# ESMS-Group-Public/FoKL-GPy

Hardware: AMD Instinct MI355X
Metric: candidate-terms/sec (basis build + Gibbs + BIC) (higher is better)
Workload: dtype f64

## Files before the change

fokl_gpy_amd/_capi.py:

```python
import ctypes
import os

import numpy as np

_HERE = os.path.dirname(os.path.abspath(__file__))
LIB_PATH = os.environ.get('FOKL_HIP_LIBRARY', os.path.join(_HERE, 'libfokl_hip.so'))

UNIQUE_ID_BYTES = 128
K_BASIS, K_GRAM, K_RESID, K_PREDICT, K_RESID_MF, K_GRAM_MFMA, K_GRAM_REDUCE = 0, 1, 2, 3, 4, 5, 6
K_INTEGRATE, K_BAND = 7, 8
K_OPTIMIZE = 9
K_OPTIMIZE_SYSTEM = 10
K_POPULATION = 11
K_RESAMPLE = 12
K_SCORE = 13
K_INFER = 14
K_DESIGN = 15
INTEGRATE_MAX_STATES = 4
RESID_TERMS_MAX_FACTORS = 32
RESID_TERMS_MAX_ORDER = 8
RESID_TERMS_LAYOUTS = ((8, 1), (16, 1), (8, 2), (4, 4), (2, 8), (8, 4), (16, 2), (4, 8))
SLOT_ONES, SLOT_Y, SLOT_FIRST_FREE = 0, 1, 2
PREDICT_NONE, PREDICT_VALU_LDS, PREDICT_VALU_GLOBAL, PREDICT_MFMA = 0, 1, 2, 3
POPULATION_COEFFICIENTS = ('none', 'registers', 'table')
# ... 106 lines not shown
    'fokl_stream_given_gauss': (c_dbl, [c_vp]),
    'fokl_stream_destroy': (None, [c_vp]),
    'fokl_stream_walk': (c_int, [c_vp, c_int, c_int, c_dbl, c_dbl, c_vp, c_vp, c_vp, c_vp]),
    'fokl_stream_tell': (c_int, [c_vp, c_vp]),
    'fokl_stream_seek': (c_int, [c_vp, c_vp]),
    'fokl_stream_hold': (c_int, [c_vp, c_vp]),
    'fokl_stream_release': (c_int, [c_vp, ctypes.c_uint64]),
    'fokl_stream_advance_floor': (c_int, [c_vp]),
    'fokl_stream_state': (c_int, [c_vp, c_vp, c_vp, c_vp, c_vp]),
    'fokl_stream_expand': (c_int, [c_vp, c_int, c_dbl, c_dbl, c_vp, c_int, c_int, c_vp, c_vp, c_vp, c_vp, c_vp]),
    'fokl_stream_stats': (c_int, [c_vp, c_vp, c_vp, c_vp, c_vp, c_vp]),
    'fokl_stream_set_helpers': (c_int, [c_vp, c_int, c_vp]),
    'fokl_stream_place_bulk': (c_int, [c_vp, c_vp, c_int]),
    'fokl_stream_fast_ln_error': (c_dbl, [c_i64]),
    'fokl_search_create': (c_int, [c_vp, c_vp, c_vp, c_vp]),
    'fokl_search_bind_spectral': (c_int, [c_vp, c_vp, c_int, c_dbl, c_int]),
    'fokl_search_hold_spectral': (c_int, [c_vp, c_int]),
    'fokl_search_set_update': (c_int, [c_vp, c_int, c_int, c_int]),
    'fokl_search_set_decide': (c_int, [c_vp, c_int, c_dbl]),
    'fokl_search_set_deterministic': (c_int, [c_vp, c_int]),
    'fokl_search_destroy': (None, [c_vp]),
    'fokl_search_error': (ctypes.c_char_p, [c_vp]),
    'fokl_search_mispredicted': (c_int, [c_vp]),
    'fokl_search_set_substage': (c_int, [c_vp, c_vp, c_int]),
    'fokl_search_speculate': (c_int, [c_vp, c_vp, c_vp, c_int]),
    'fokl_search_drop_speculation': (c_int, [c_vp]),
    'fokl_search_spectral': (c_int, [c_vp, c_vp, c_int, c_vp, c_int, c_vp]),
    'fokl_search_spectral_from': (c_int, [c_vp, c_vp, c_int, c_vp, c_int, c_vp, c_int, c_vp]),
    'fokl_spectrum_done': (c_int, [c_vp]),
    'fokl_spectrum_wait': (c_int, [c_vp, c_vp, c_vp, c_vp]),
    'fokl_spectrum_release': (None, [c_vp, c_vp]),
    'fokl_spectrum_retain': (c_int, [c_vp, c_vp]),
    'fokl_search_model_begin': (c_int, [c_vp, c_vp, c_int, c_vp, c_int, c_vp, c_vp, c_vp, c_int, c_vp, c_vp]),
    'fokl_search_model_commit': (c_int, [c_vp, c_vp, c_vp, c_dbl, c_int, c_vp]),
    'fokl_run_create': (c_int, [c_vp, c_vp, c_vp]),
    'fokl_run_set_update': (c_int, [c_vp, c_int, c_int, c_int]),
    'fokl_run_search': (c_int, [c_vp, c_vp]),
    'fokl_run_result': (c_int, [c_vp, c_vp, c_vp, c_vp, c_vp, c_vp]),
    'fokl_run_arrays': (c_int, [c_vp, c_vp, c_vp, c_vp, c_vp, c_vp, c_vp]),
    'fokl_run_error': (ctypes.c_char_p, [c_vp]),
    'fokl_run_destroy': (None, [c_vp]),
    'fokl_search_score': (c_int, [c_vp, c_vp, c_dbl, c_dbl, c_int, c_int, c_vp]),
    'fokl_outcome_info': (c_int, [c_vp, c_vp, c_vp]),
    'fokl_outcome_spectrum': (c_int, [c_vp, c_vp, c_vp]),
    'fokl_outcome_chain_ready': (c_int, [c_vp]),
    'fokl_outcome_draws': (c_int, [c_vp, c_vp, c_vp]),
    'fokl_outcome_intercept_scale': (c_int, [c_vp, c_vp, c_vp]),
    'fokl_outcome_new_term_stats': (c_int, [c_vp, c_vp, c_vp, c_int, c_int, c_int, c_vp, c_vp]),
    'fokl_outcome_release': (None, [c_vp, c_vp]),
    'fokl_outcome_drop': (None, [c_vp, c_vp]),
    'fokl_search_verify': (c_int, [c_vp, c_int]),
    'fokl_search_register_forecast': (c_int, [c_vp, c_vp, c_int, c_vp, c_dbl]),
    'fokl_search_clear_forecasts': (None, [c_vp]),
    'fokl_search_likely_first_tests': (c_int, [c_vp, c_vp, c_int, c_dbl, c_vp, c_vp, c_vp]),
    'fokl_search_stats': (c_int, [c_vp, c_vp, c_int]),
    'fokl_search_trace': (c_i64, [c_vp, c_vp, c_i64]),
    'fokl_search_kill_tests': (c_int, [c_vp, c_vp, c_vp]),
    'fokl_finish_tape_blocks': (c_int, [c_int, c_int, c_vp, c_vp, c_vp, c_vp, c_int, c_int, c_int, c_vp]),
    'fokl_gibbs_chain_from_finished_tape': (c_int, [c_vp, c_vp, c_int, c_dbl, c_dbl, c_dbl, c_dbl, c_dbl, c_int, c_vp,
                                                    c_vp, c_vp, c_vp, c_int, c_vp, c_vp, c_vp, c_vp]),
    'fokl_gibbs_chain_segments_host': (c_int, [c_vp, c_vp, c_int, c_dbl, c_dbl, c_dbl, c_dbl, c_dbl, c_int, c_vp, c_vp,
                                               c_vp, c_vp, c_int, c_vp, c_vp, c_vp, c_vp, c_int, c_int, c_vp]),
    'fokl_rng_normals': (c_int, [c_vp, c_vp, c_vp, c_vp, c_i64, c_vp]),
    'fokl_rng_gammas': (c_int, [c_vp, c_vp, c_vp, c_vp, c_dbl, c_dbl, c_i64, c_vp]),
    'fokl_gp_integrate': (c_int, [c_int, c_int, c_i64, c_vp, c_vp, c_vp, c_vp, c_vp, c_vp, c_vp, c_vp, c_vp, c_int, c_int,
                                  c_dbl, c_vp, c_vp]),
    'fokl_gp_integrate_ensemble': (c_int, [c_vp, c_int, c_int, c_int, c_i64, c_vp, c_vp, c_vp, c_vp, c_vp, c_vp, c_vp, c_vp,
                                           c_vp, c_vp, c_int, c_int, c_dbl, c_vp, c_int, c_int, c_vp, c_vp, c_vp]),
    'fokl_simulate_ensemble': (c_int, [c_vp, c_vp, c_int, c_vp, c_vp, c_vp, c_vp]),
    'fokl_simulate_report': (c_int, [c_vp, c_vp]),
    'fokl_simulate_adaptive': (c_int, [c_vp, c_vp, c_int, c_dbl, c_vp, c_int, c_int, c_vp, c_vp, c_vp, c_vp, c_vp, c_vp, c_vp, c_vp, c_vp,
                                       c_vp]),
# ... 1276 lines not shown
        mean_w, flag = job.wait()
        return job.fetch_w(), np.array(mean_w), bool(flag[0])
    finally:
        job.release()



_OPS_SIGS = (('reserve_slots', [c_vp, c_int]),
             ('build_terms', [c_vp, c_vp, c_int, c_vp]),
             ('gram', [c_vp, c_vp, c_int, c_vp, c_int, c_vp, c_int, c_int]),
             ('gram_launch', [c_vp, c_vp, c_int, c_vp, c_int, c_int]),
             ('gram_fetch', [c_vp, c_vp, c_i64]),
             ('gram_ready', [c_vp]),
             ('bic_resid', [c_vp, c_vp, c_int, c_vp, c_vp, c_int]),
             ('bic_resid_launch', [c_vp, c_vp, c_int, c_vp]),
             ('bic_resid_fetch', [c_vp, c_vp, c_int]),
             ('bic_resid_terms_launch', [c_vp, c_vp, c_int, c_vp]))
_OPS_TYPES = {name: ctypes.CFUNCTYPE(c_int, *args) for name, args in _OPS_SIGS}


class _BackendOps(ctypes.Structure):
    _fields_ = [('ctx', c_vp)] + [(name, c_vp) for name, _ in _OPS_SIGS] + [('kernel_id', c_i32)]


class _RunParams(ctypes.Structure):
    _fields_ = [(name, c_i32) for name in (
        'm', 'n_phis', 'way3', 'tolerance', 'gimmie', 'draws', 'half0', 'lookahead', 'lookahead_native', 'foresight',
        'speculate_across', 'forecast_early', 'forecast_polls', 'matrix_free', 'update_from', 'update_depth',
        'update_lookahead', 'head_start', 'slot_capacity')]


RUN_STATS = ('terms_physical', 'substages', 'forecasts_used', 'forecasts_early', 'resid_matrix_free', 't_resid',
             'phase_prepare', 'phase_model', 'phase_statistics', 'phase_tests', 'phase_wrap_up')


def backend_ops(backend, kernel_id):
    lib = load()
    ops = _BackendOps()
    ops.kernel_id = int(kernel_id)
    ctx = getattr(backend, 'ctx', None)
    if isinstance(ctx, DeviceContext):
        ops.ctx = ctx._h
        for name, _ in _OPS_SIGS:
            setattr(ops, name, ctypes.cast(getattr(lib, 'fokl_' + name), c_vp).value)
        return ops, (ctx,)
    pending, raised = {}, []

    def arr(ptr, count, ctype, dtype):
        return np.array(np.ctypeslib.as_array(ctypes.cast(ptr, ctypes.POINTER(ctype * count)).contents), dtype=dtype)

    def guard(fn):
        def call(*args):
            try:
                fn(*args)
                return 0
            except BaseException as exc:
                raised.append(exc)
                return -3
        return call

    def out(ptr, values):
        values = np.ascontiguousarray(values, dtype=np.float64).reshape(-1)
        ctypes.memmove(ptr, values.ctypes.data, values.nbytes)

    def reserve_slots(_c, n):
        backend.reserve_slots(int(n))

    def build_terms(_c, terms, T, slots):
        sl = arr(slots, T, ctypes.c_int32, np.int32)
        m = pending['m']
        backend.build_terms(arr(terms, T * m, ctypes.c_int32, np.int32).reshape(T, m), [int(v) for v in sl])

    def gram(_c, rows, nr, cols, nc, dst, _path, allreduce):
        out(dst, backend.gram([int(v) for v in arr(rows, nr, ctypes.c_int32, np.int32)],
                              [int(v) for v in arr(cols, nc, ctypes.c_int32, np.int32)], bool(allreduce)))

    def gram_launch(_c, rows, nr, cols, nc, allreduce):
        pending['gram'] = backend.gram([int(v) for v in arr(rows, nr, ctypes.c_int32, np.int32)],
                                       [int(v) for v in arr(cols, nc, ctypes.c_int32, np.int32)], bool(allreduce))

    def gram_fetch(_c, dst, count):
        block = pending.pop('gram')
        assert block.size == count
        out(dst, block)

    def bic_resid(_c, slots, nc, betahat, dst, allreduce):
        out(dst, backend.bic_resid([int(v) for v in arr(slots, nc, ctypes.c_int32, np.int32)],
                                   arr(betahat, nc, ctypes.c_double, np.float64), bool(allreduce)))

    def bic_resid_launch(_c, slots, nc, betahat):
        pending['resid'] = backend.bic_resid([int(v) for v in arr(slots, nc, ctypes.c_int32, np.int32)],
                                             arr(betahat, nc, ctypes.c_double, np.float64), False)

    def bic_resid_fetch(_c, dst, _allreduce):
        out(dst, pending.pop('resid'))

    table = dict(reserve_slots=reserve_slots, build_terms=build_terms, gram=gram, gram_launch=gram_launch,
                 gram_fetch=gram_fetch, bic_resid=bic_resid, bic_resid_launch=bic_resid_launch,
                 bic_resid_fetch=bic_resid_fetch)
    keep = [pending, raised]
    for name, fn in table.items():
        cb = _OPS_TYPES[name](guard(fn))
        keep.append(cb)
        setattr(ops, name, ctypes.cast(cb, c_vp).value)
    return ops, tuple(keep)


class NativeRun:

    def __init__(self, backend, kernel_id, **params):
        self._lib = load()
        self._h = None
        self._ops, self._keep = backend_ops(backend, kernel_id)
        if isinstance(self._keep[0], dict):
            self._keep[0]['m'] = int(params['m'])
        self._prm = _RunParams(**{k: int(v) for k, v in params.items()})
        self.m = int(params['m'])
        h = c_vp(0)
        _check(self._lib.fokl_run_create(ctypes.byref(self._ops), ctypes.byref(self._prm), ctypes.byref(h)))
        self._h = h
        self._reraise()

    def _reraise(self):
        raised = self._keep[1] if isinstance(self._keep[0], dict) else None
        if raised:
            exc = raised[0]
            del raised[:]
            raise exc

    def set_update(self, from_columns, depth, lookahead):
        _check(self._lib.fokl_run_set_update(self._h, int(from_columns), int(depth), int(lookahead)))

    def search(self, native_search):
        rc = self._lib.fokl_run_search(self._h, native_search._h)
        self._reraise()
        if rc != 0:
            native_search._checked(rc)
        return self

    def result(self):
        rows, n_evs, subs = c_i32(0), c_i32(0), c_i32(0)
        best, last = c_vp(0), c_vp(0)
        _check(self._lib.fokl_run_result(self._h, ctypes.byref(rows), ctypes.byref(n_evs), ctypes.byref(subs),
                                         ctypes.byref(best), ctypes.byref(last)))
        mtx = np.zeros((max(rows.value, 0), self.m), dtype=np.int32)
        evs = np.zeros(n_evs.value)
        sizes = np.zeros(max(subs.value, 1), dtype=np.int32)
        stats = np.zeros(16)
        total = self._lib.fokl_run_arrays(self._h, _ptr(mtx) if mtx.size else None, _ptr(evs) if evs.size else None,
                                          _ptr(sizes), None, None, _ptr(stats))
        mean_abs, rel_std = np.zeros(max(total, 1)), np.zeros(max(total, 1))
        self._lib.fokl_run_arrays(self._h, None, None, None, _ptr(mean_abs), _ptr(rel_std), None)
        per, at = [], 0
        for size in sizes[:subs.value]:
            per.append(dict(mean_abs=mean_abs[at:at + size].copy(), rel_std=rel_std[at:at + size].copy()))
            at += int(size)
        return (mtx.astype(np.float64), evs, per, best.value, last.value, dict(zip(RUN_STATS, stats[:len(RUN_STATS)])))

    def close(self):
        if self._h is not None and self._h:
            self._lib.fokl_run_destroy(self._h)
            self._h = None

    def __del__(self):
        try:
            self.close()
        except Exception:
            pass


class _FirstTrialStruct(ctypes.Structure):
    _fields_ = [(name, ctypes.c_void_p) for name in ('trial', 'slope', 'moved', 'pooled', 'ft', 'ft_sums', 'phi_t', 'a_t', 'z',
                                                      'status', 'descent')]


class _SystemStruct(ctypes.Structure):
    _fields_ = [('n_members', c_int), ('n_states', c_int), ('n_steps', c_i64), ('h', c_dbl), ('n_forcing_cols', c_int),
                ('forcing', c_vp), ('n_norm_forcing', c_int), ('n_norm', c_int), ('norm_src', c_vp), ('norm_lo', c_vp),
                ('norm_span', c_vp), ('n_forcing_factors', c_int), ('n_factors', c_int), ('fac_norm', c_vp), ('fac_kind', c_vp),
                ('fac_row', c_vp), ('fac_degree', c_vp), ('n_spline_rows', c_int), ('spline_table', c_vp), ('n_bern_rows', c_int),
                ('bern_table', c_vp), ('n_entries', c_int), ('entries', c_vp), ('entry_begin', c_vp), ('entry_count', c_vp),
                ('constant', c_vp), ('n_coef', c_int), ('coef', c_vp), ('y0', c_vp), ('box', c_vp)]


class _ControlProblemStruct(ctypes.Structure):
    _fields_ = [('n_controls', c_int), ('n_segments', c_int), ('seg_first', c_vp), ('norm_control', c_vp), ('ctl_lo', c_vp),
                ('ctl_width', c_vp), ('ref', c_vp), ('track_weight', c_vp), ('terminal_weight', c_vp), ('limit_lo', c_vp),
                ('limit_hi', c_vp), ('limit_weight', c_dbl), ('move_weight', c_vp), ('previous', c_vp), ('has_previous', c_int),
                ('n_starts', c_int), ('z0', c_vp), ('max_iter', c_int), ('tol', c_dbl)]

# ... 933 lines not shown
```

fokl_gpy_amd/csrc/fokl_run.cpp:

```cpp
#include <algorithm>
#include <chrono>
#include <cmath>
#include <cstdint>
#include <cstring>
#include <map>
#include <memory>
#include <string>
#include <vector>

#include "../../include/fokl_hip_internal.h"

extern void fokl_set_global_error(const std::string &msg);

namespace {

inline double now_s()
{
    return 1e-9 * (double)std::chrono::duration_cast<std::chrono::nanoseconds>(
                      std::chrono::steady_clock::now().time_since_epoch())
                      .count();
}

using Gram = std::shared_ptr<std::vector<double>>;

// ... 134 lines not shown
    for (int r = 0; r < vm; ++r) {
        const double *b = block.data() + (size_t)r * block_ld;
        double *row = o + (size_t)(n_prev + r) * L;
        for (int j = 0; j < n_prev; ++j) {
            const double v = b[block_kept[(size_t)j]];
            row[j] = v;
            o[(size_t)j * L + n_prev + r] = v;
        }
        for (int c = 0; c < vm; ++c) row[n_prev + c] = b[over + c];
        row[A2] = o[(size_t)A2 * L + n_prev + r] = b[over + vm];
    }
    return out;
}

}

struct fokl_run {
    fokl_backend_ops ops{};
    fokl_run_params prm{};
    Slots pool;
    Patterns patterns;
    std::vector<double> base;
    Ahead ahead;
    bool have_next = false;
    int next_stage = 0;
    std::vector<int32_t> next_indvec;
    std::vector<int32_t> mtx;
    int mtx_rows = 0;
    std::vector<double> evs;
    fokl_outcome *best_model = nullptr, *last_model = nullptr;
    std::vector<double> stat_mean_abs, stat_rel_std;
    std::vector<int32_t> stat_sizes;
    double stats[FOKL_RUN_STATS] = {};
    std::string error;
};

namespace {

int run_fail(fokl_run *r, int code, const std::string &msg)
{
    if (r) r->error = msg;
    fokl_set_global_error(msg);
    return code;
}

enum RunStat {
    R_TERMS_PHYSICAL, R_SUBSTAGES, R_FORECASTS_USED, R_FORECASTS_EARLY, R_RESID_MATRIX_FREE, R_T_RESID, R_PHASE_PREPARE,
    R_PHASE_MODEL, R_PHASE_STATISTICS, R_PHASE_TESTS, R_PHASE_WRAP_UP, R_COUNT
};
static_assert(R_COUNT <= FOKL_RUN_STATS, "fokl_run_stats: grow FOKL_RUN_STATS");

int matrix_free_pay_from(const fokl_backend_ops &ops, const std::vector<int32_t> &terms, int rows, int m)
{
    static const int layouts[8][2] = {{8, 1}, {16, 1}, {8, 2}, {4, 4}, {2, 8}, {8, 4}, {16, 2}, {4, 8}};
    if (!ops.bic_resid_terms_launch || rows < 1) return -1;
    int max_order = 0;
    for (int t = 0; t < rows; ++t) {
        int nz = 0;
        for (int j = 0; j < m; ++j) {
            const int v = terms[(size_t)t * m + j];
            nz += v != 0;
            max_order = std::max(max_order, v);
        }
        if (nz > 2) return -1;
    }
    if (max_order == 0) return -1;
    if (ops.kernel_id != 0 && max_order > 8) return -1;
    int inputs = 0, deepest = 0;
    for (int j = 0; j < m; ++j) {
        std::vector<int32_t> seen;
        for (int t = 0; t < rows; ++t) {
            const int v = terms[(size_t)t * m + j];
            if (v != 0 && std::find(seen.begin(), seen.end(), v) == seen.end()) seen.push_back(v);
        }
        inputs += !seen.empty();
        deepest = std::max(deepest, (int)seen.size());
    }
    int best = -1;
    for (auto &l : layouts)
        if (inputs <= l[0] && deepest <= l[1] && (best < 0 || l[0] * l[1] < best)) best = l[0] * l[1];
    if (best < 0) return -1;
    return ops.kernel_id != 0 ? 0 : (int)(3.5 * best);
}

static const bool g_build_at_start = !(std::getenv("FOKL_BUILD_AHEAD_AT") && std::strcmp(std::getenv("FOKL_BUILD_AHEAD_AT"), "model") == 0);

struct Loop {
    fokl_run *r;
    fokl_search *s;
    const fokl_backend_ops &ops;
    const fokl_run_params &prm;
    int m;
    std::vector<int32_t> damtx;
    std::vector<int32_t> model_slots;
    std::vector<int> keep;
    Gram gram;
    int gram_A = 0;
    std::vector<int32_t> active_slots;
    int A = 0, vm = 0, n_prev = 0, vm_next = -1;
    Gram cur;
    std::vector<int32_t> terms_arr;
    int terms_pay_from = 0;
    std::map<std::vector<int64_t>, int64_t> term_ids;
    std::vector<SpectrumRef> early;
    std::vector<std::vector<int32_t>> early_keys;
    std::vector<int32_t> predicted_kills;
    bool have_predicted = false;
    Ahead ahead;
    bool have_coming = false;
    int coming_stage = 0;
    std::vector<int32_t> coming_indvec;
    struct Forecast {
        std::vector<int32_t> key;
        SpectrumRef sp;
    };
    std::vector<Forecast> forecasts;
    std::vector<fokl_outcome *> outcomes, retiring;
    int rc_cb = FOKL_OK;

    Loop(fokl_run *run, fokl_search *search) : r(run), s(search), ops(run->ops), prm(run->prm), m(run->prm.m) {}

    void release(SpectrumRef &sp)
    {
        if (sp.h) fokl_spectrum_release(s, sp.h);
        sp.h = nullptr;
        sp.gram.reset();
    }

    std::vector<int32_t> columns_without(int count, const std::vector<int32_t> &removed) const
    {
        std::vector<int32_t> out;
        for (int c = 0; c < count; ++c)
            if (std::find(removed.begin(), removed.end(), c) == removed.end()) out.push_back(c);
        return out;
    }

    int fetch_block(Ahead &a)
    {
        if (a.pending) {
            const int nc = a.over + a.T + 1;
            a.block.resize((size_t)a.T * nc);
            const int rc = ops.gram_fetch(ops.ctx, a.block.data(), (int64_t)a.T * nc);
            if (rc != FOKL_OK) return rc;
            a.pending = false;
        }
        return FOKL_OK;
    }

    int build_ahead(const std::vector<int32_t> &indvec, const std::vector<int32_t> &active, Ahead *out)
    {
        Ahead a;
// ... 243 lines not shown
                return rc;
            std::vector<int> kept((size_t)n_prev);
            for (int i = 0; i < n_prev; ++i) kept[(size_t)i] = i;
            cur = extend_gram(*gram, gram_A, keep, block, T, (int)cols.size(), kept, n_prev);
        }
        vm = (int)(vecs.size() / (size_t)m);
        damtx.insert(damtx.end(), vecs.begin(), vecs.end());
        const int dam = (int)(damtx.size() / (size_t)m);
        if ((rc = set_active_terms()) != FOKL_OK) return rc;
        active_slots.assign(1, FOKL_SLOT_ONES);
        active_slots.insert(active_slots.end(), model_slots.begin(), model_slots.end());
        active_slots.insert(active_slots.end(), new_slots.begin(), new_slots.end());
        A = (int)active_slots.size();
        vm_next = have_coming ? (int)(arrangements(coming_indvec).size() / (size_t)m) : -1;
        early.clear();
        early_keys.clear();
        have_predicted = false;
        bool guessed = false;
        std::vector<std::pair<int, bool>> then;
        if (vm > 0 && A > 1) then.push_back({A - 1, false});
        if (prm.lookahead > 0 && spectral_job.h && fokl_spectrum_done(spectral_job.h)) {
            if ((rc = guess_first_tests(spectral_job.h, vm, NAN, true, &then)) != FOKL_OK) return rc;
            guessed = true;
        }
        lap(R_PHASE_PREPARE);

        std::vector<int32_t> idx((size_t)A);
        for (int i = 0; i < A; ++i) idx[(size_t)i] = i;
        std::vector<int32_t> then_sizes, then_model;
        for (auto &p : then) {
            then_sizes.push_back(p.first);
            then_model.push_back(p.second ? 1 : 0);
        }
        fokl_spectrum *spectrum = nullptr;
        fokl_tape *tape = nullptr;
        if ((rc = fokl_search_model_begin(s, cur->data(), A + 1, idx.data(), A, spectral_job.h, then_sizes.data(),
                                          then_model.data(), (int)then_sizes.size(), &spectrum, &tape)) != FOKL_OK)
            return rc;
        if (g_build_at_start && have_coming && prm.foresight > 0) {
            if ((rc = build_ahead_columns(coming_indvec, &ahead)) != FOKL_OK) {
                fokl_spectrum_release(s, spectrum);
                return rc;
            }
        }
        const double *buffer = nullptr;
        int p1_check = 0;
        if ((rc = fokl_spectrum_wait(s, spectrum, &buffer, &p1_check)) != FOKL_OK) {
            fokl_spectrum_release(s, spectrum);
            return rc;
        }
        const double *betahat = buffer + 2 * (size_t)A;
        if (!terms_arr.empty() && A >= terms_pay_from) {
            rc = ops.bic_resid_terms_launch(ops.ctx, terms_arr.data() + m, A - 1, betahat);
            R->stats[R_RESID_MATRIX_FREE] += 1;
        } else {
            rc = ops.bic_resid_launch(ops.ctx, active_slots.data(), A, betahat);
        }
        if (rc == FOKL_OK && ahead.built && !ahead.valid) rc = launch_ahead_gram(active_slots, &ahead);
        if (rc == FOKL_OK && !guessed && prm.lookahead > 0 && vm > 0) {
            rc = guess_first_tests(spectrum, vm, NAN, false);
            guessed = rc == FOKL_OK;
        }
        fokl_outcome *full = nullptr;
        if (rc == FOKL_OK) rc = fokl_search_model_commit(s, spectrum, tape, (*cur)[(size_t)A * (A + 1) + A], vm, &full);
        if (rc != FOKL_OK) {
            fokl_spectrum_release(s, spectrum);
            return rc;
        }
        release(spectral_job);
        outcomes.push_back(full);
        auto forecast_now = [&]() {
            if (!(g_build_at_start && prm.forecast_early && ahead.valid && ahead.pending && have_predicted && ops.gram_ready &&
                  forecasts.empty()))
                return;
            if (!ops.gram_ready(ops.ctx)) return;
            foresee(predicted_kills.data(), (int)predicted_kills.size());
            if (rc_cb == FOKL_OK) R->stats[R_FORECASTS_EARLY] += 1;
        };
        forecast_now();
        if (rc_cb != FOKL_OK) return rc_cb;
        {
            const double t0 = now_s();
            double mom[2] = {0, 0};
            if ((rc = ops.bic_resid_fetch(ops.ctx, mom, 0)) != FOKL_OK) return rc;
            R->stats[R_T_RESID] += now_s() - t0;
            forecast_now();
            if (rc_cb != FOKL_OK) return rc_cb;
            double ev_model = 0;
            if ((rc = fokl_search_score(s, full, mom[0], mom[1], n_prev, 0, &ev_model)) != FOKL_OK) return rc;
        }
        fokl_outcome *best = full;
        fokl_outcome_view view{};
        if ((rc = fokl_outcome_info(s, full, &view)) != FOKL_OK) return rc;
        double ev = view.ev;
        lap(R_PHASE_MODEL);

        if (!guessed && prm.lookahead > 0) {
            fokl_spectrum *own = nullptr;
            if ((rc = fokl_outcome_spectrum(s, full, &own)) != FOKL_OK) return rc;
            rc = guess_first_tests(own, vm, view.siglik, false);
            fokl_spectrum_release(s, own);
            if (rc != FOKL_OK) return rc;
        }
        release_retired();
        if (have_coming && prm.foresight > 0 && !ahead.valid && !ahead.built) {
            if ((rc = build_ahead(coming_indvec, active_slots, &ahead)) != FOKL_OK) return rc;
        }
        if (prm.forecast_early && ahead.valid && ahead.pending && have_predicted && ops.gram_ready && forecasts.empty()) {
            for (int polls = prm.forecast_polls; polls > 0 && !fokl_outcome_chain_ready(full); --polls)
                if (ops.gram_ready(ops.ctx)) {
                    foresee(predicted_kills.data(), (int)predicted_kills.size());
                    if (rc_cb != FOKL_OK) return rc_cb;
                    R->stats[R_FORECASTS_EARLY] += 1;
                    break;
                }
        }
// ... 174 lines not shown
        if (r->have_next) {
            Loop head(r, nullptr);
            rc = head.build_ahead(r->next_indvec, {FOKL_SLOT_ONES}, &r->ahead);
        }
    }
    if (rc != FOKL_OK) {
        delete r;
        return rc;
    }
    *out = r;
    return FOKL_OK;
}

extern "C" int fokl_run_set_update(fokl_run *r, int from_columns, int depth, int lookahead)
{
    if (!r) return run_fail(nullptr, FOKL_ERR_ARG, "fokl_run_set_update: null run");
    r->prm.update_from = from_columns;
    r->prm.update_depth = depth;
    r->prm.update_lookahead = lookahead;
    return FOKL_OK;
}

extern "C" int fokl_run_search(fokl_run *r, fokl_search *search)
{
    if (!r || !search) return run_fail(r, FOKL_ERR_ARG, "fokl_run_search: null pointer");
    Loop loop(r, search);
    const int rc = loop.run();
    if (rc != FOKL_OK) {
        for (auto &e : loop.early) loop.release(e);
        for (auto &f : loop.forecasts) loop.release(f.sp);
        for (fokl_outcome *o : loop.outcomes) fokl_outcome_drop(search, o);
        for (fokl_outcome *o : loop.retiring) fokl_outcome_drop(search, o);
        if (loop.ahead.valid && loop.ahead.pending) (void)loop.fetch_block(loop.ahead);
    }
    return rc;
}

extern "C" int fokl_run_result(const fokl_run *r, int32_t *mtx_rows, int32_t *evs_count, int32_t *substages,
                               fokl_outcome **best_model, fokl_outcome **last_model)
{
    if (!r || !mtx_rows || !evs_count || !substages || !best_model || !last_model)
        return run_fail(nullptr, FOKL_ERR_ARG, "fokl_run_result: null pointer");
    *mtx_rows = r->mtx_rows;
    *evs_count = (int32_t)r->evs.size();
    *substages = (int32_t)r->stat_sizes.size();
    *best_model = r->best_model;
    *last_model = r->last_model;
    return FOKL_OK;
}

extern "C" int fokl_run_arrays(const fokl_run *r, int32_t *mtx, double *evs, int32_t *stat_sizes, double *stat_mean_abs,
                               double *stat_rel_std, double *stats)
{
    if (!r) return run_fail(nullptr, FOKL_ERR_ARG, "fokl_run_arrays: null run");
    if (mtx) std::memcpy(mtx, r->mtx.data(), sizeof(int32_t) * r->mtx.size());
    if (evs) std::memcpy(evs, r->evs.data(), sizeof(double) * r->evs.size());
    if (stat_sizes) std::memcpy(stat_sizes, r->stat_sizes.data(), sizeof(int32_t) * r->stat_sizes.size());
    if (stat_mean_abs) std::memcpy(stat_mean_abs, r->stat_mean_abs.data(), sizeof(double) * r->stat_mean_abs.size());
    if (stat_rel_std) std::memcpy(stat_rel_std, r->stat_rel_std.data(), sizeof(double) * r->stat_rel_std.size());
    if (stats) std::memcpy(stats, r->stats, sizeof(double) * FOKL_RUN_STATS);
    return (int)r->stat_mean_abs.size();
}

extern "C" const char *fokl_run_error(const fokl_run *r) { return r ? r->error.c_str() : ""; }

extern "C" void fokl_run_destroy(fokl_run *r)
{
    if (!r) return;
    if (r->ahead.valid && r->ahead.pending) {
        r->ahead.block.resize((size_t)r->ahead.T * (size_t)(r->ahead.over + r->ahead.T + 1));
        (void)r->ops.gram_fetch(r->ops.ctx, r->ahead.block.data(), (int64_t)r->ahead.block.size());
    }
    delete r;
}
```

fokl_gpy_amd/csrc/fokl_search.cpp:

```cpp
#include <algorithm>
#include <atomic>
#include <chrono>
#include <cmath>
#include <cstdint>
#include <cstdio>
#include <cstdlib>
#include <cstring>
#include <deque>
#include <map>
#include <memory>
#include <mutex>
#include <string>
#include <thread>
#include <vector>

#include <immintrin.h>

#include "../../include/fokl_hip_internal.h"
#include "fokl_spin.h"

extern void fokl_set_global_error(const std::string &msg);

extern "C" __attribute__((visibility("hidden"))) int fokl_gibbs_chain_from_raw_blocks(
    const double *lamb, const double *qty, int p1, double b, double btau, double dtd, double sigsqd0, double tausqd0,
// ... 1633 lines not shown

extern "C" int fokl_search_hold_spectral(fokl_search *s, int hold)
{
    if (!s) return fail(nullptr, FOKL_ERR_ARG, "fokl_search_hold_spectral: null search");
    s->dspec_hold = hold != 0;
    if (!s->dspec_hold) flush_spectra(s);
    return FOKL_OK;
}

extern "C" int fokl_spectrum_done(fokl_spectrum *h) { return h && spectrum_done(reinterpret_cast<Spectrum *>(h)) ? 1 : 0; }

extern "C" int fokl_spectrum_wait(fokl_search *s, fokl_spectrum *h, const double **buffer, int *p1)
{
    if (!s || !h) return fail(s, FOKL_ERR_ARG, "fokl_spectrum_wait: null pointer");
    Spectrum *sp = reinterpret_cast<Spectrum *>(h);
    const int rc = wait_spectrum(s, sp);
    if (buffer) *buffer = sp->buf;
    if (p1) *p1 = sp->p1;
    return rc;
}

extern "C" int fokl_spectrum_retain(fokl_search *s, fokl_spectrum *h)
{
    if (!s || !h) return fail(s, FOKL_ERR_ARG, "fokl_spectrum_retain: null pointer");
    reinterpret_cast<Spectrum *>(h)->refs += 1;
    return FOKL_OK;
}

extern "C" void fokl_spectrum_release(fokl_search *s, fokl_spectrum *h)
{
    if (s && h) unref(s, reinterpret_cast<Spectrum *>(h));
}

extern "C" int fokl_search_model_begin(fokl_search *s, const double *gram, int ld, const int32_t *idx, int p1,
                                       fokl_spectrum *given, const int32_t *then_sizes, const int32_t *then_model,
                                       int then_count, fokl_spectrum **spectrum_out, fokl_tape **tape_out)
{
    if (!s || !gram || !idx || p1 < 1 || !spectrum_out || !tape_out)
        return fail(s, FOKL_ERR_ARG, "fokl_search_model_begin: bad arguments");
    Tape *t = tape_for(s, p1, true);
    if (!t) return FOKL_ERR_STATE;
    std::vector<std::pair<int, bool>> want;
    for (int i = 0; i < then_count; ++i) want.push_back({then_sizes[i], then_model[i] != 0});
    speculate(s, want);
    Spectrum *sp = reinterpret_cast<Spectrum *>(given);
    if (sp)
        sp->refs += 1;
    else
        sp = submit_spectrum(s, gram, ld, idx, p1);
    if (!sp) {
        unref(s, t);
        return FOKL_ERR_STATE;
    }
    flush_spectra(s);
    const int rc = wait_spectrum(s, sp);
    if (rc != FOKL_OK) {
        unref(s, sp);
        unref(s, t);
        return rc;
    }
    *spectrum_out = reinterpret_cast<fokl_spectrum *>(sp);
    *tape_out = reinterpret_cast<fokl_tape *>(t);
    return FOKL_OK;
}

extern "C" int fokl_search_model_commit(fokl_search *s, fokl_spectrum *spectrum, fokl_tape *tape, double dtd, int new_terms,
                                        fokl_outcome **out)
{
    if (!s || !spectrum || !tape || !out || new_terms < 0)
        return fail(s, FOKL_ERR_ARG, "fokl_search_model_commit: null pointer or negative count");
    Spectrum *sp = reinterpret_cast<Spectrum *>(spectrum);
    Outcome *o = commit(s, sp, reinterpret_cast<Tape *>(tape), dtd, false, new_terms);
    unref(s, sp);
    if (!o) return FOKL_ERR_STATE;
    *out = reinterpret_cast<fokl_outcome *>(o);
    return FOKL_OK;
}

extern "C" int fokl_search_score(fokl_search *s, fokl_outcome *h, double s1, double s2, int n_prev, int kill, double *ev)
{
    if (!s || !h || !ev) return fail(s, FOKL_ERR_ARG, "fokl_search_score: null pointer");
    Outcome *o = reinterpret_cast<Outcome *>(h);
    const int p1 = o->spec->p1;
    o->ev = same_model_same_ev(s, o->spec->idx.data(), p1, ev_from_moments(s, s1, s2, p1));
    o->siglik = s->last_siglik;
    o->s1 = s1;
    o->s2 = s2;
    o->trace_index = record(s, p1, n_prev, o->ev, kill != 0);
    *ev = o->ev;
    return FOKL_OK;
}

extern "C" int fokl_outcome_info(fokl_search *s, fokl_outcome *h, fokl_outcome_view *view)
{
    if (!s || !h || !view) return fail(s, FOKL_ERR_ARG, "fokl_outcome_info: null pointer");
// ... 833 lines not shown
```

fokl_gpy_amd/engine.py:

```python
import collections
import itertools
import threading
import math
import os
import time

import numpy as np
from scipy.linalg import eigh as _eigh

from . import _capi

SLOT_ONES, SLOT_Y, SLOT_FIRST_FREE = _capi.SLOT_ONES, _capi.SLOT_Y, _capi.SLOT_FIRST_FREE
from .host_pipeline import (
    HostPipeline, ShardedSpectralJob, GibbsOutcome, EagerOutcome, NativeOutcome, NativeSpectrum, Misprediction, ModelSize,
    chain_engine_for, spectral_engine_for,
    close_chain_engines, drop_spare_buffers, _mark, _flush_marks, _cpu_budget, _thread_plan, _thread_spares,
    _place_host_threads, _SPARES)



def distinct_arrangements(indvec):
    cur = sorted(float(v) for v in indvec)
    n = len(cur)
    rows = [tuple(cur)]
# ... 1035 lines not shown
        return ahead['block']

    @staticmethod
    def _extend_gram(gram, keep, block, block_kept, over):
        A = gram.shape[0] - 1
        n_prev, vm = len(keep), block.shape[0]
        A2 = n_prev + vm
        out = np.empty((A2 + 1, A2 + 1))
        out[:n_prev, :n_prev] = gram[np.ix_(keep, keep)]
        out[:n_prev, A2] = out[A2, :n_prev] = gram[keep, A]
        out[A2, A2] = gram[A, A]
        cross = block[:, block_kept]
        out[n_prev:A2, :n_prev] = cross
        out[:n_prev, n_prev:A2] = cross.T
        out[n_prev:A2, n_prev:A2] = block[:, over:over + vm]
        out[n_prev:A2, A2] = out[A2, n_prev:A2] = block[:, over + vm]
        return out

    def _run_native(self):
        nrun, self._nrun = self._nrun, None
        if self._update_args is not None:
            nrun.set_update(*self._update_args)
        try:
            nrun.search(self.native)
            mtx, evs, per_substage, best_h, last_h, st = nrun.result()
        finally:
            nrun.close()
        self.substage_stats = per_substage
        for key in ('terms_physical', 'substages', 'forecasts_used', 'resid_matrix_free'):
            self.stats[key] += int(st[key])
        self.stats['forecasts_early'] = self.stats.get('forecasts_early', 0) + int(st['forecasts_early'])
        self.stats['t_resid'] += st['t_resid']
        self.stats['substage_loop'] = 'native'
        phase = self.stats.setdefault('phases', dict(prepare=0.0, model=0.0, statistics=0.0, tests=0.0, wrap_up=0.0))
        for key in phase:
            phase[key] += st['phase_' + key]
        betas = NativeOutcome(self, self.native, best_h)
        last = betas if last_h == best_h else NativeOutcome(self, self.native, last_h)
        self._outcomes = [betas] if last is betas else [betas, last]
        if self.chain_engine is not None and hasattr(self.chain_engine, 'flush'):
            self.chain_engine.flush()
        return self._finish(betas, mtx, evs, last)

    def _run(self):
        if getattr(self, '_nrun', None) is not None:
            if self.native is not None:
                return self._run_native()
            self._nrun.close()
            self._nrun = None
        m, n = self.m, self.n
        draws = self.draws
        half1 = int(math.ceil(draws / 2 + 1))
        half0 = int(math.ceil(draws / 2))

        model_slots = []
        damtx = np.zeros((0, m))
        head = getattr(self, '_head', None)
        self._head = None
        if head is not None:
            base = head[0]
        else:
            base = self.backend.gram([SLOT_ONES, SLOT_Y], [SLOT_ONES, SLOT_Y], self.allreduce)
        gram = np.array(base, dtype=np.float64)
        keep = [0]

        evs = np.array([])
# ... 235 lines not shown
```

include/fokl_hip_internal.h:

```cpp
#ifndef FOKL_HIP_INTERNAL_H
#define FOKL_HIP_INTERNAL_H

#include <stddef.h>

#include "fokl_hip.h"

#ifdef __cplusplus
extern "C" {
#endif


#define FOKL_SEGMENT_BLOCKS 256
#define FOKL_SEGMENT_DOUBLES 79872
#define FOKL_ROW_LEAD (1ull << 63)
#define FOKL_SOURCE_X1_HALF (1ull << 63)
#define FOKL_SOURCE_GIVEN ((1ull << 62) - 1)
#define FOKL_GAMMA_FINAL_VALUE (~0ull)
#define FOKL_PRESTATE_WORDS 640
#define FOKL_PRESTATE_BLOCKS 32
typedef struct fokl_stream fokl_stream;
typedef struct fokl_tape_row {
    uint64_t start;
    uint64_t lead_source;
    uint64_t gamma[2];
// ... 98 lines not shown
    int32_t half0;
    int32_t aic;
    int32_t lookahead, foresight;
    int32_t speculation_max;
    int32_t tentative_tapes, test_rewinds;
    int32_t device_chain_columns;
    int32_t finish_threads;
    int32_t flip_guess;
    int32_t device_rows;
} fokl_search_params;
int fokl_search_create(fokl_host_pool *pool, fokl_dchain *dchain, const fokl_search_params *params, fokl_search **out);
typedef struct fokl_dspectral fokl_dspectral;
int fokl_search_bind_spectral(fokl_search *search, fokl_dspectral *engine, int max_columns, double slack, int lookahead);
int fokl_search_hold_spectral(fokl_search *search, int hold);
int fokl_search_set_update(fokl_search *search, int from_columns, int depth, int lookahead);
int fokl_search_set_decide(fokl_search *search, int mode, double tolerance);
int fokl_search_set_deterministic(fokl_search *search, int on);
void fokl_search_destroy(fokl_search *search);
const char *fokl_search_error(const fokl_search *search);
int fokl_search_mispredicted(const fokl_search *search);
int fokl_search_set_substage(fokl_search *search, const int64_t *term_ids, int columns);
int fokl_search_speculate(fokl_search *search, const int32_t *sizes, const int32_t *is_model, int count);
int fokl_search_drop_speculation(fokl_search *search);
int fokl_search_spectral(fokl_search *search, const double *gram, int ld, const int32_t *idx, int p1, fokl_spectrum **out);
int fokl_search_spectral_from(fokl_search *search, const double *gram, int ld, const int32_t *idx, int p1,
                              fokl_spectrum *parent, int parent_pos, fokl_spectrum **out);
int fokl_spectrum_done(fokl_spectrum *spectrum);
int fokl_spectrum_wait(fokl_search *search, fokl_spectrum *spectrum, const double **buffer, int *p1);
int fokl_spectrum_retain(fokl_search *search, fokl_spectrum *spectrum);
void fokl_spectrum_release(fokl_search *search, fokl_spectrum *spectrum);
int fokl_search_model_begin(fokl_search *search, const double *gram, int ld, const int32_t *idx, int p1,
                            fokl_spectrum *given, const int32_t *then_sizes, const int32_t *then_model, int then_count,
                            fokl_spectrum **spectrum_out, fokl_tape **tape_out);
int fokl_search_model_commit(fokl_search *search, fokl_spectrum *spectrum, fokl_tape *tape, double dtd, int new_terms,
                             fokl_outcome **out);
int fokl_search_score(fokl_search *search, fokl_outcome *outcome, double sum_r, double sum_r2, int n_prev, int kill,
                      double *ev);
typedef struct fokl_outcome_view {
    const double *spectrum;
    const int32_t *idx;
    double ev, siglik, intercept_scale;
    int32_t p1, on_device;
} fokl_outcome_view;
int fokl_outcome_info(fokl_search *search, fokl_outcome *outcome, fokl_outcome_view *view);
int fokl_outcome_spectrum(fokl_search *search, fokl_outcome *outcome, fokl_spectrum **out);
int fokl_outcome_chain_ready(fokl_outcome *outcome);
int fokl_outcome_draws(fokl_search *search, fokl_outcome *outcome, const double **w);
int fokl_outcome_intercept_scale(fokl_search *search, fokl_outcome *outcome, double *scale);
int fokl_outcome_new_term_stats(fokl_search *search, fokl_outcome *outcome, const int32_t *cols, int count, int half0,
                                int half1, double *mean_abs, double *rel_std);
void fokl_outcome_release(fokl_search *search, fokl_outcome *outcome);
void fokl_outcome_drop(fokl_search *search, fokl_outcome *outcome);
int fokl_search_verify(fokl_search *search, int block);
int fokl_search_register_forecast(fokl_search *search, const int32_t *key, int key_count, fokl_spectrum *spectrum,
                                  double dtd);
void fokl_search_clear_forecasts(fokl_search *search);
int fokl_search_likely_first_tests(fokl_search *search, fokl_spectrum *spectrum, int n_new, double siglik,
                                   int32_t *columns_out, int32_t *accepted_out, int *count);
int fokl_search_stats(const fokl_search *search, double *values, int count);
int64_t fokl_search_trace(const fokl_search *search, double *records, int64_t capacity);
typedef struct fokl_kill_tests_args {
    const double *gram;
    const int32_t *columns;
    const double *mean_abs, *rel_std;
    const int32_t *slots;
    fokl_outcome *best;
// ... 18 lines not shown
    int (*reserve_slots)(void *ctx, int n_slots);
    int (*build_terms)(void *ctx, const int32_t *terms, int T, const int32_t *slots);
    int (*gram)(void *ctx, const int32_t *row_slots, int nr, const int32_t *col_slots, int nc, double *out, int path,
                int allreduce);
    int (*gram_launch)(void *ctx, const int32_t *row_slots, int nr, const int32_t *col_slots, int nc, int allreduce);
    int (*gram_fetch)(void *ctx, double *out, int64_t count);
    int (*gram_ready)(void *ctx);
    int (*bic_resid)(void *ctx, const int32_t *slots, int nc, const double *betahat, double *out, int allreduce);
    int (*bic_resid_launch)(void *ctx, const int32_t *slots, int nc, const double *betahat);
    int (*bic_resid_fetch)(void *ctx, double *out, int allreduce);
    int (*bic_resid_terms_launch)(void *ctx, const int32_t *terms, int n_terms, const double *betahat);
    int32_t kernel_id;
} fokl_backend_ops;
typedef struct fokl_run_params {
    int32_t m, n_phis;
    int32_t way3, tolerance, gimmie;
    int32_t draws, half0;
    int32_t lookahead, lookahead_native, foresight, speculate_across;
    int32_t forecast_early, forecast_polls;
    int32_t matrix_free;
    int32_t update_from, update_depth, update_lookahead;
    int32_t head_start;
    int32_t slot_capacity;
} fokl_run_params;
#define FOKL_RUN_STATS 16
typedef struct fokl_run fokl_run;
int fokl_run_create(const fokl_backend_ops *ops, const fokl_run_params *params, fokl_run **out);
int fokl_run_set_update(fokl_run *run, int from_columns, int depth, int lookahead);
int fokl_run_search(fokl_run *run, fokl_search *search);
int fokl_run_result(const fokl_run *run, int32_t *mtx_rows, int32_t *evs_count, int32_t *substages,
                    fokl_outcome **best_model, fokl_outcome **last_model);
int fokl_run_arrays(const fokl_run *run, int32_t *mtx, double *evs, int32_t *stat_sizes, double *stat_mean_abs,
                    double *stat_rel_std, double *stats);
const char *fokl_run_error(const fokl_run *run);
void fokl_run_destroy(fokl_run *run);


int fokl_dchain_create(int device, int slots, fokl_dchain **out);
void fokl_dchain_destroy(fokl_dchain *engine);
int fokl_dchain_submit(fokl_dchain *engine, int p1, int draws, const double *lamb, const double *qty, double b,
                       double btau, double dtd, double sigsqd0, double tausqd0, const double *normals,
                       const int32_t *lead, const double *gam_sig, const double *gam_tau, const int32_t *progress,
                       const int32_t *block_done, int block, int finished, int stat_first, int64_t *ticket,
                       const double **stats_area);
int fokl_dchain_prestate_ring(fokl_dchain *engine, uint32_t **ring, int *entries);
int fokl_dchain_bind_stream(fokl_dchain *engine, const fokl_stream *stream);
int fokl_dchain_submit_rows(fokl_dchain *engine, int p1, int draws, const double *lamb, const double *qty, double b,
                            double btau, double dtd, double sigsqd0, double tausqd0, double astar, double atau_star,
                            const fokl_tape_row *rows, const double *gam_sig, const double *gam_tau,
                            const int32_t *progress, const uint64_t *span, int stat_first, int64_t *ticket,
                            const double **stats_area);
int fokl_dchain_stream_stats(fokl_dchain *engine, int64_t *segments_made, int64_t *rows_jobs);
int fokl_dchain_poll(fokl_dchain *engine, int64_t ticket);
int fokl_dchain_flush(fokl_dchain *engine);
int fokl_dchain_wait(fokl_dchain *engine, int64_t ticket, double *stats_out);
int fokl_dchain_fetch_w(fokl_dchain *engine, int64_t ticket, double *w_out);
int fokl_dchain_release(fokl_dchain *engine, int64_t ticket);
int fokl_dchain_try_release(fokl_dchain *engine, int64_t ticket);
int fokl_dchain_stats(fokl_dchain *engine, double *busy_seconds, int64_t *issued, int64_t *launches, int64_t *staged);
int fokl_dchain_recuts(fokl_dchain *engine, int64_t *recuts);

#define FOKL_DSPECTRAL_MAX_COLUMNS 192
int fokl_dspectral_create(int device, fokl_dspectral **out);
void fokl_dspectral_destroy(fokl_dspectral *engine);
int fokl_dspectral_max_columns(void);
int fokl_dspectral_set_signs(fokl_dspectral *engine, int canonical);
// ... 353 lines not shown
```

Before: 571,000.

## Split model begin into request/wait and reorder model substage launches

Adds a non-blocking model request so the native run loop can build look-ahead columns while the spectral decomposition is still pending, and only then waits on it. After the spectrum arrives it commits the chain first, places first-test orders, and then launches the BIC residual and the look-ahead Gram, so the orders reach the device sooner. It also records per-substage timestamps that are exposed to Python, and adds cleanup of a pending residual fetch and look-ahead slots on error. The reordering changes which work overlaps with which, and could delay the residual kernel behind order placement.

```diff
diff --git a/fokl_gpy_amd/_capi.py b/fokl_gpy_amd/_capi.py
--- a/fokl_gpy_amd/_capi.py
+++ b/fokl_gpy_amd/_capi.py
@@ -162,12 +162,15 @@
     'fokl_spectrum_release': (None, [c_vp, c_vp]),
     'fokl_spectrum_retain': (c_int, [c_vp, c_vp]),
     'fokl_search_model_begin': (c_int, [c_vp, c_vp, c_int, c_vp, c_int, c_vp, c_vp, c_vp, c_int, c_vp, c_vp]),
+    'fokl_search_model_request': (c_int, [c_vp, c_vp, c_int, c_vp, c_int, c_vp, c_vp, c_vp, c_int, c_vp, c_vp]),
+    'fokl_search_model_abandon': (None, [c_vp, c_vp, c_vp]),
     'fokl_search_model_commit': (c_int, [c_vp, c_vp, c_vp, c_dbl, c_int, c_vp]),
     'fokl_run_create': (c_int, [c_vp, c_vp, c_vp]),
     'fokl_run_set_update': (c_int, [c_vp, c_int, c_int, c_int]),
     'fokl_run_search': (c_int, [c_vp, c_vp]),
     'fokl_run_result': (c_int, [c_vp, c_vp, c_vp, c_vp, c_vp, c_vp]),
     'fokl_run_arrays': (c_int, [c_vp, c_vp, c_vp, c_vp, c_vp, c_vp, c_vp]),
+    'fokl_run_order': (c_int, [c_vp, c_vp, c_int]),
     'fokl_run_error': (ctypes.c_char_p, [c_vp]),
     'fokl_run_destroy': (None, [c_vp]),
     'fokl_search_score': (c_int, [c_vp, c_vp, c_dbl, c_dbl, c_int, c_int, c_vp]),
@@ -1510,6 +1513,7 @@
 
 RUN_STATS = ('terms_physical', 'substages', 'forecasts_used', 'forecasts_early', 'resid_matrix_free', 't_resid',
              'phase_prepare', 'phase_model', 'phase_statistics', 'phase_tests', 'phase_wrap_up')
+RUN_ORDER = ('k1_ahead', 'g2_wait_begun', 'g2_arrived', 'chain_submitted', 'orders_placed', 'k3_launched', 'ahead_gram_launched')
 
 
 def backend_ops(backend, kernel_id):
@@ -1573,9 +1577,16 @@
     def bic_resid_fetch(_c, dst, _allreduce):
         out(dst, pending.pop('resid'))
 
+    def bic_resid_terms_launch(_c, terms, n_terms, betahat):
+        m = pending['m']
+        pending['resid'] = backend.bic_resid_terms_launch(arr(terms, n_terms * m, ctypes.c_int32, np.int32).reshape(n_terms, m),
+                                                          arr(betahat, n_terms + 1, ctypes.c_double, np.float64))
+
     table = dict(reserve_slots=reserve_slots, build_terms=build_terms, gram=gram, gram_launch=gram_launch,
                  gram_fetch=gram_fetch, bic_resid=bic_resid, bic_resid_launch=bic_resid_launch,
                  bic_resid_fetch=bic_resid_fetch)
+    if hasattr(backend, 'bic_resid_terms_launch'):
+        table['bic_resid_terms_launch'] = bic_resid_terms_launch
     keep = [pending, raised]
     for name, fn in table.items():
         cb = _OPS_TYPES[name](guard(fn))
@@ -1633,7 +1644,11 @@
         for size in sizes[:subs.value]:
             per.append(dict(mean_abs=mean_abs[at:at + size].copy(), rel_std=rel_std[at:at + size].copy()))
             at += int(size)
-        return (mtx.astype(np.float64), evs, per, best.value, last.value, dict(zip(RUN_STATS, stats[:len(RUN_STATS)])))
+        st = dict(zip(RUN_STATS, stats[:len(RUN_STATS)]))
+        order = np.full((max(self._lib.fokl_run_order(self._h, None, 0), 1), len(RUN_ORDER)), np.nan)
+        rows = self._lib.fokl_run_order(self._h, _ptr(order), order.shape[0])
+        st['substage_order'] = [{k: (None if np.isnan(v) else float(v)) for k, v in zip(RUN_ORDER, row)} for row in order[:rows]]
+        return (mtx.astype(np.float64), evs, per, best.value, last.value, st)
 
     def close(self):
         if self._h is not None and self._h:
diff --git a/fokl_gpy_amd/csrc/fokl_run.cpp b/fokl_gpy_amd/csrc/fokl_run.cpp
--- a/fokl_gpy_amd/csrc/fokl_run.cpp
+++ b/fokl_gpy_amd/csrc/fokl_run.cpp
@@ -190,6 +190,7 @@
     std::vector<double> stat_mean_abs, stat_rel_std;
     std::vector<int32_t> stat_sizes;
     double stats[FOKL_RUN_STATS] = {};
+    std::vector<double> order;
     std::string error;
 };
 
@@ -242,6 +243,11 @@
 }
 
 static const bool g_build_at_start = !(std::getenv("FOKL_BUILD_AHEAD_AT") && std::strcmp(std::getenv("FOKL_BUILD_AHEAD_AT"), "model") == 0);
+
+static const bool g_k3_before_orders = std::getenv("FOKL_MODEL_ORDER") && std::strcmp(std::getenv("FOKL_MODEL_ORDER"), "k3first") == 0;
+
+enum OrderStamp { O_K1_AHEAD, O_WAIT_BEGUN, O_G2_ARRIVED, O_CHAIN, O_ORDERS, O_K3, O_AHEAD_GRAM, O_COUNT };
+static_assert(O_COUNT == FOKL_RUN_ORDER_STAMPS, "fokl_run_order: FOKL_RUN_ORDER_STAMPS columns");
 
 struct Loop {
     fokl_run *r;
@@ -275,6 +281,7 @@
     std::vector<Forecast> forecasts;
     std::vector<fokl_outcome *> outcomes, retiring;
     int rc_cb = FOKL_OK;
+    bool resid_launched = false;
 
     Loop(fokl_run *run, fokl_search *search) : r(run), s(search), ops(run->ops), prm(run->prm), m(run->prm.m) {}
 
@@ -584,43 +591,62 @@
             then_sizes.push_back(p.first);
             then_model.push_back(p.second ? 1 : 0);
         }
+        double stamp[FOKL_RUN_ORDER_STAMPS];
+        for (double &v : stamp) v = NAN;
+        if (guessed) stamp[O_ORDERS] = now_s();
         fokl_spectrum *spectrum = nullptr;
         fokl_tape *tape = nullptr;
-        if ((rc = fokl_search_model_begin(s, cur->data(), A + 1, idx.data(), A, spectral_job.h, then_sizes.data(),
-                                          then_model.data(), (int)then_sizes.size(), &spectrum, &tape)) != FOKL_OK)
+        if ((rc = fokl_search_model_request(s, cur->data(), A + 1, idx.data(), A, spectral_job.h, then_sizes.data(),
+                                            then_model.data(), (int)then_sizes.size(), &spectrum, &tape)) != FOKL_OK)
             return rc;
         if (g_build_at_start && have_coming && prm.foresight > 0) {
             if ((rc = build_ahead_columns(coming_indvec, &ahead)) != FOKL_OK) {
-                fokl_spectrum_release(s, spectrum);
+                fokl_search_model_abandon(s, spectrum, tape);
                 return rc;
             }
+            stamp[O_K1_AHEAD] = now_s();
         }
         const double *buffer = nullptr;
         int p1_check = 0;
+        stamp[O_WAIT_BEGUN] = now_s();
         if ((rc = fokl_spectrum_wait(s, spectrum, &buffer, &p1_check)) != FOKL_OK) {
-            fokl_spectrum_release(s, spectrum);
+            fokl_search_model_abandon(s, spectrum, tape);
             return rc;
         }
+        stamp[O_G2_ARRIVED] = now_s();
+        fokl_outcome *full = nullptr;
+        if ((rc = fokl_search_model_commit(s, spectrum, tape, (*cur)[(size_t)A * (A + 1) + A], vm, &full)) != FOKL_OK) return rc;
+        stamp[O_CHAIN] = now_s();
+        release(spectral_job);
+        outcomes.push_back(full);
         const double *betahat = buffer + 2 * (size_t)A;
+        auto place_orders = [&]() -> int {
+            if (guessed || prm.lookahead <= 0 || vm <= 0) return FOKL_OK;
+            fokl_spectrum *own = nullptr;
+            int rcg = fokl_outcome_spectrum(s, full, &own);
+            if (rcg != FOKL_OK) return rcg;
+            rcg = guess_first_tests(own, vm, NAN, false);
+            fokl_spectrum_release(s, own);
+            guessed = rcg == FOKL_OK;
+            stamp[O_ORDERS] = now_s();
+            return rcg;
+        };
+        if (!g_k3_before_orders && (rc = place_orders()) != FOKL_OK) return rc;
         if (!terms_arr.empty() && A >= terms_pay_from) {
             rc = ops.bic_resid_terms_launch(ops.ctx, terms_arr.data() + m, A - 1, betahat);
             R->stats[R_RESID_MATRIX_FREE] += 1;
         } else {
             rc = ops.bic_resid_launch(ops.ctx, active_slots.data(), A, betahat);
         }
-        if (rc == FOKL_OK && ahead.built && !ahead.valid) rc = launch_ahead_gram(active_slots, &ahead);
-        if (rc == FOKL_OK && !guessed && prm.lookahead > 0 && vm > 0) {
-            rc = guess_first_tests(spectrum, vm, NAN, false);
-            guessed = rc == FOKL_OK;
-        }
-        fokl_outcome *full = nullptr;
-        if (rc == FOKL_OK) rc = fokl_search_model_commit(s, spectrum, tape, (*cur)[(size_t)A * (A + 1) + A], vm, &full);
-        if (rc != FOKL_OK) {
-            fokl_spectrum_release(s, spectrum);
-            return rc;
-        }
-        release(spectral_job);
-        outcomes.push_back(full);
+        if (rc != FOKL_OK) return rc;
+        resid_launched = true;
+        stamp[O_K3] = now_s();
+        if (g_k3_before_orders && (rc = place_orders()) != FOKL_OK) return rc;
+        if (ahead.built && !ahead.valid) {
+            if ((rc = launch_ahead_gram(active_slots, &ahead)) != FOKL_OK) return rc;
+            stamp[O_AHEAD_GRAM] = now_s();
+        }
+        R->order.insert(R->order.end(), stamp, stamp + FOKL_RUN_ORDER_STAMPS);
         auto forecast_now = [&]() {
             if (!(g_build_at_start && prm.forecast_early && ahead.valid && ahead.pending && have_predicted && ops.gram_ready &&
                   forecasts.empty()))
@@ -634,6 +660,7 @@
         {
             const double t0 = now_s();
             double mom[2] = {0, 0};
+            resid_launched = false;
             if ((rc = ops.bic_resid_fetch(ops.ctx, mom, 0)) != FOKL_OK) return rc;
             R->stats[R_T_RESID] += now_s() - t0;
             forecast_now();
@@ -874,6 +901,13 @@
         for (fokl_outcome *o : loop.outcomes) fokl_outcome_drop(search, o);
         for (fokl_outcome *o : loop.retiring) fokl_outcome_drop(search, o);
         if (loop.ahead.valid && loop.ahead.pending) (void)loop.fetch_block(loop.ahead);
+        if (loop.resid_launched) {
+            double dummy[2];
+            (void)r->ops.bic_resid_fetch(r->ops.ctx, dummy, 0);
+            loop.resid_launched = false;
+        }
+        r->pool.give(loop.ahead.slots);
+        loop.ahead = Ahead();
     }
     return rc;
 }
@@ -904,6 +938,15 @@
     return (int)r->stat_mean_abs.size();
 }
 
+extern "C" int fokl_run_order(const fokl_run *r, double *stamps, int capacity)
+{
+    if (!r) return run_fail(nullptr, FOKL_ERR_ARG, "fokl_run_order: null run");
+    const int rows = (int)(r->order.size() / FOKL_RUN_ORDER_STAMPS);
+    if (stamps && capacity > 0)
+        std::memcpy(stamps, r->order.data(), sizeof(double) * FOKL_RUN_ORDER_STAMPS * (size_t)std::min(rows, capacity));
+    return rows;
+}
+
 extern "C" const char *fokl_run_error(const fokl_run *r) { return r ? r->error.c_str() : ""; }
 
 extern "C" void fokl_run_destroy(fokl_run *r)
diff --git a/fokl_gpy_amd/csrc/fokl_search.cpp b/fokl_gpy_amd/csrc/fokl_search.cpp
--- a/fokl_gpy_amd/csrc/fokl_search.cpp
+++ b/fokl_gpy_amd/csrc/fokl_search.cpp
@@ -1689,12 +1689,12 @@
     if (s && h) unref(s, reinterpret_cast<Spectrum *>(h));
 }
 
-extern "C" int fokl_search_model_begin(fokl_search *s, const double *gram, int ld, const int32_t *idx, int p1,
-                                       fokl_spectrum *given, const int32_t *then_sizes, const int32_t *then_model,
-                                       int then_count, fokl_spectrum **spectrum_out, fokl_tape **tape_out)
+extern "C" int fokl_search_model_request(fokl_search *s, const double *gram, int ld, const int32_t *idx, int p1,
+                                         fokl_spectrum *given, const int32_t *then_sizes, const int32_t *then_model,
+                                         int then_count, fokl_spectrum **spectrum_out, fokl_tape **tape_out)
 {
     if (!s || !gram || !idx || p1 < 1 || !spectrum_out || !tape_out)
-        return fail(s, FOKL_ERR_ARG, "fokl_search_model_begin: bad arguments");
+        return fail(s, FOKL_ERR_ARG, "fokl_search_model_request: bad arguments");
     Tape *t = tape_for(s, p1, true);
     if (!t) return FOKL_ERR_STATE;
     std::vector<std::pair<int, bool>> want;
@@ -1710,14 +1710,34 @@
         return FOKL_ERR_STATE;
     }
     flush_spectra(s);
-    const int rc = wait_spectrum(s, sp);
-    if (rc != FOKL_OK) {
-        unref(s, sp);
-        unref(s, t);
-        return rc;
-    }
     *spectrum_out = reinterpret_cast<fokl_spectrum *>(sp);
     *tape_out = reinterpret_cast<fokl_tape *>(t);
+    return FOKL_OK;
+}
+
+extern "C" void fokl_search_model_abandon(fokl_search *s, fokl_spectrum *spectrum, fokl_tape *tape)
+{
+    if (!s) return;
+    if (spectrum) unref(s, reinterpret_cast<Spectrum *>(spectrum));
+    if (tape) unref(s, reinterpret_cast<Tape *>(tape));
+}
+
+extern "C" int fokl_search_model_begin(fokl_search *s, const double *gram, int ld, const int32_t *idx, int p1,
+                                       fokl_spectrum *given, const int32_t *then_sizes, const int32_t *then_model,
+                                       int then_count, fokl_spectrum **spectrum_out, fokl_tape **tape_out)
+{
+    if (!s || !gram || !idx || p1 < 1 || !spectrum_out || !tape_out)
+        return fail(s, FOKL_ERR_ARG, "fokl_search_model_begin: bad arguments");
+    fokl_spectrum *spectrum = nullptr;
+    fokl_tape *tape = nullptr;
+    int rc = fokl_search_model_request(s, gram, ld, idx, p1, given, then_sizes, then_model, then_count, &spectrum, &tape);
+    if (rc != FOKL_OK) return rc;
+    if ((rc = wait_spectrum(s, reinterpret_cast<Spectrum *>(spectrum))) != FOKL_OK) {
+        fokl_search_model_abandon(s, spectrum, tape);
+        return rc;
+    }
+    *spectrum_out = spectrum;
+    *tape_out = tape;
     return FOKL_OK;
 }
 
diff --git a/fokl_gpy_amd/engine.py b/fokl_gpy_amd/engine.py
--- a/fokl_gpy_amd/engine.py
+++ b/fokl_gpy_amd/engine.py
@@ -1091,6 +1091,7 @@
         self.stats['forecasts_early'] = self.stats.get('forecasts_early', 0) + int(st['forecasts_early'])
         self.stats['t_resid'] += st['t_resid']
         self.stats['substage_loop'] = 'native'
+        self.stats['substage_order'] = st['substage_order']
         phase = self.stats.setdefault('phases', dict(prepare=0.0, model=0.0, statistics=0.0, tests=0.0, wrap_up=0.0))
         for key in phase:
             phase[key] += st['phase_' + key]
diff --git a/include/fokl_hip_internal.h b/include/fokl_hip_internal.h
--- a/include/fokl_hip_internal.h
+++ b/include/fokl_hip_internal.h
@@ -154,6 +154,10 @@
 int fokl_search_model_begin(fokl_search *search, const double *gram, int ld, const int32_t *idx, int p1,
                             fokl_spectrum *given, const int32_t *then_sizes, const int32_t *then_model, int then_count,
                             fokl_spectrum **spectrum_out, fokl_tape **tape_out);
+int fokl_search_model_request(fokl_search *search, const double *gram, int ld, const int32_t *idx, int p1,
+                              fokl_spectrum *given, const int32_t *then_sizes, const int32_t *then_model, int then_count,
+                              fokl_spectrum **spectrum_out, fokl_tape **tape_out);
+void fokl_search_model_abandon(fokl_search *search, fokl_spectrum *spectrum, fokl_tape *tape);
 int fokl_search_model_commit(fokl_search *search, fokl_spectrum *spectrum, fokl_tape *tape, double dtd, int new_terms,
                              fokl_outcome **out);
 int fokl_search_score(fokl_search *search, fokl_outcome *outcome, double sum_r, double sum_r2, int n_prev, int kill,
@@ -238,6 +242,8 @@
                     fokl_outcome **best_model, fokl_outcome **last_model);
 int fokl_run_arrays(const fokl_run *run, int32_t *mtx, double *evs, int32_t *stat_sizes, double *stat_mean_abs,
                     double *stat_rel_std, double *stats);
+#define FOKL_RUN_ORDER_STAMPS 7
+int fokl_run_order(const fokl_run *run, double *stamps, int capacity);
 const char *fokl_run_error(const fokl_run *run);
 void fokl_run_destroy(fokl_run *run);
 
```

New measurement: 603,200 (median of 6 runs). +5.6%, better.
